# CrystalSixone/VLN-MAGIC

Measured on AMD Instinct MI355X. Metric: trajectory-steps/sec (whole node), MAGIC-S R2R pretrain, higher is better.
Workload: dtype bf16

## Files before the change

include/magic_hip.h:

```cpp
#ifndef MAGIC_HIP_H
#define MAGIC_HIP_H
#ifdef __cplusplus
extern "C" {
#endif

#define MAGIC_OK 0
#define MAGIC_ERR_ARG (-1)
#define MAGIC_ERR_LAUNCH (-2)
#define MAGIC_ERR_UNSUPPORTED (-3)

int magic_abi_version(void);
int magic_build_id(char* out, int len);
int magic_device_info(int* cu_count, int* clock_khz, char* arch, int arch_len);

int magic_gemm(int dtype, int layout, int batch, int nh, int M, int N, int K,
               const void* A, int lda, long long sAb, long long sAh,
               const void* B, int ldb, long long sBb, long long sBh,
               void* C, int ldc, long long sCb, long long sCh, int c_f32, int accumulate,
               const float* bias, int epilogue, const void* aux, int ldaux,
               const void* residual, int ldr, void* C2, int ldc2,
               float alpha, int splitk, float* bias_grad, void* stream);
int magic_gemm_set_big(int mode);
#define MAGIC_GEMM_FORM_PLAIN 0x1
#define MAGIC_GEMM_FORM_XCD 0x2
// ... 129 lines not shown
                      const float* dist, float* dsprel_w, float* dsprel_b, void* stream);
int magic_head_mean_fwd(int dtype, int B, int nh, long long inner, const void* P, float* out, void* stream);
int magic_head_mean_bwd(int B, int nh, long long inner, const float* g, float* dP, int accumulate, void* stream);

int magic_attn_supported(int dtype, int Nq, int Nk, int backward);
int magic_attn_fwd(int dtype, int B, int nh, int Nq, int Nk, const void* q, int ldq, const void* k, const void* v, int ldkv,
                   void* P, int ldp, void* ctx, int H, float scale, const unsigned char* kmask, const float* dist,
                   const float* sprel_w, const float* sprel_b,
                   const void* drop_seed, float drop_p, unsigned drop_site, void* Pd, void* stream);
int magic_attn_bwd(int dtype, int B, int nh, int Nq, int Nk, const void* q, int ldq, const void* k, const void* v, int ldkv,
                   const void* P, int ldp, const void* dctx, int H, float scale, const float* dP_init,
                   void* dq, int lddq, void* dk, void* dv, int lddkv,
                   const float* dist, float* dsprel_w, float* dsprel_b,
                   const void* drop_seed, float drop_p, unsigned drop_site, void* stream);
int magic_attn_bwd_ks(int dtype, int B, int nh, int Nq, int Nk, const void* q, int ldq, const void* k, const void* v, int ldkv,
                      const void* P, int ldp, const void* o, const void* dctx, int H, float scale,
                      void* dq, int lddq, void* dk, void* dv, int lddkv, int accumulate_kv,
                      const void* drop_seed, float drop_p, unsigned drop_site, void* stream);

int magic_lndot_fwd(int dtype, int M, int H, const void* Y, const float* gamma, const float* beta, float eps,
                    const float* w2, const float* b2, float* logit, void* stream);
int magic_lndot_bwd_blocks(int M);
int magic_lndot_bwd(int dtype, int M, int H, const void* Y, const float* gamma, const float* beta, float eps,
                    const float* w2, const float* dlogit, void* dZ, float* dgamma, float* dbeta, float* dw2, float* db2,
                    float* part, void* stream);

int magic_ce_rows(int dtype, int M, int N, const void* logits, int ld, const int* labels, int ignore_index,
                  float coef, const float* row_w, float* loss_row, void* dlogits, int ldd, int accumulate,
                  float* w_out, float w_rate, void* stream);
int magic_softkl_rows(int dtype, int M, int N, const void* logits, int ld, const float* targets, int ldt, float coef,
                      const float* row_w , float* loss_row, void* dlogits, int ldd,
                      void* stream);

int magic_kd_rows(int M, int N, const float* s, const float* t, int ld, float temperature, const float* w, float norm,
                  float coef, const float* coef_dev, float* loss_row, float* ds, int accumulate, void* stream);
int magic_kd_cols_parts(long long outer, int C, long long inner);
int magic_kd_cols(int dtype, long long outer, int C, long long inner, const void* s, long long s_stride, const void* t,
                  long long t_stride, float temperature, const float* w, float norm, float coef, float* loss_part, int n_parts,
                  void* ds, void* stream);
int magic_nav_act(int B, int K, const float* logits, int ld, const unsigned char* cand, int ldc, const unsigned char* mode,
                  const void* draws, float expl_max_ratio, int* action, float* stop_prob, float* entropy, void* stream);
int magic_mse(int dtype, int g_f32, long long outer, long long inner, const void* s, long long s_stride, const void* t,
              long long t_stride, const float* w, long long rows_per_w, float norm, float coef, const float* coef_dev, float* loss, void* ds,
              long long g_stride, int accumulate, void* stream);
typedef struct {
  int g_f32; long long outer, inner; const void* s; long long s_stride; const void* t; long long t_stride;
  const float* w; long long rows_per_w; float norm, coef; const float* coef_dev; float* loss; void* ds; long long g_stride; int accumulate;
  const int* valid_dev; const float* norm_dev; long long valid_mod;
} magic_mse_desc;
int magic_mse_multi(int dtype, int n, const magic_mse_desc* d, void* stream);
int magic_kd_emb_supported(int dtype, int Hs, int Ht);
int magic_kd_emb(int dtype, int n, const magic_mse_desc* d, int Hs, int Ht, const int* M, const void* const* W, const float* const* b,
                 void* const* d_acc, void* stream);
int magic_cfp_loss(int dtype, int B, int H, const void* a0, const void* a1, const void* a2, const void* txt, float temperature, float coef,
                   float* rows, void* d0, void* d1, void* d2, void* dtxt, float* part, int* counter, void* stream);

int magic_mlm_eval_supported(int dtype, int H);
int magic_mlm_eval_ws_need(int dtype, int nm, int V, int H);
int magic_mlm_eval(int dtype, int nm, int V, int H, const void* hm, const void* W, int ldw, const float* bias,
                   const int* labels, int ignore_index, void* ws, float* loss_row, int* hit_row, void* stream);
int magic_eval_rows(int dtype, int M, int N, const void* logits, int ld, const int* labels, int ignore_index,
                    const float* targets, int ldt, float* loss_row, int* hit_row, void* stream);
int magic_cfp_eval(int dtype, int B, int H, const void* a, const void* txt, float temperature,
                   float* loss_row, int* hit_row, void* stream);
int magic_eval_accum(int M, const float* loss_row, const int* hit_row, void* acc, int slot, void* stream);

int magic_csr_gather(int dtype, int n_out, int H, const void* src, const int* ptr, const int* idx, const float* w,
                     void* out, int accumulate, void* stream);
int magic_pano_fuse_fwd(int dtype, int N, int V, int H, const void* x, const int* lens, const float* wf, const float* bf,
                        void* fused, float* probs, const void* P, int nh, int inner, float* pmean, void* stream);
typedef struct {
  int B, K, Vp, use_gate;
  const float *g_raw, *l_raw, *fuse_raw; const unsigned char *gmask, *lmask; const int* fsrc; const unsigned char* bwmask;
  float *gl, *ll, *fl;
  const int *glab, *llab; int ignore_index; float coef;
  float *rows, *dgl, *dll, *dfl;
  const float* t_fused; float w_rate; int pad_; float* w_out;
  float T, kd_norm, kd_coef, pad2_; const float* kd_coef_dev; float* kd_rows;
} magic_sap_loss_params;
int magic_sap_fuse_loss(const void* params, int nbytes, void* stream);
int magic_pano_fuse_bwd_blocks(int N);
int magic_pano_fuse_bwd(int dtype, int N, int V, int H, const void* x, const float* probs, const float* wf, const void* dfused,
                        void* dx, float* dwf, float* dbf, void* stream);
int magic_sap_fuse_fwd(int B, int K, int Vp, const float* g_raw, const float* l_raw, const float* fuse_raw,
                       const unsigned char* gmask, const unsigned char* lmask, const int* fsrc, const unsigned char* bwmask,
                       int use_gate, float* gl, float* ll, float* fl, void* stream);
int magic_sap_fuse_bwd(int B, int K, int Vp, const float* g_raw, const float* l_raw, const float* fuse_raw,
                       const unsigned char* gmask, const unsigned char* lmask, const int* fsrc, const unsigned char* bwmask,
                       int use_gate, const float* dgl, const float* dll, const float* dfl,
                       float* dg_raw, float* dl_raw, float* dfuse_raw, void* stream);

int magic_step_rng(unsigned long long base_seed, unsigned* counter, float rw_temp, int* seed_out, float* rw_out, float* zero_me,
                   float* scale_state, float growth, float backoff, int interval, void* stream);
int magic_seed_scale(const float* scale_dev);
int magic_loss_assemble(const float* rows, int n_rows, const float* row_w, float row_scale, const float* kd_rows, int n_kd,
                        float* slots, const float* rw, float alpha, int has_kd, float* out, void* stream);

int magic_rowgate_fwd(int dtype, int M, int H, int mode, const void* x, const void* e, const float* wx, const float* we,
                      const float* b0, const float* b1, float* out_s, void* out, float* gsave, void* stream);
int magic_rowgate_bwd(int dtype, int M, int H, int mode, const void* x, const void* e, const float* wx, const float* we, const float* gsave,
                      const float* dy, const void* dout, void* dx, void* de, float* dwx, float* dwe, float* db0, float* db1, void* stream);

int magic_sumsq(long long n, const float* g, float* out, void* stream);
int magic_adamw(long long n, float* p, float* g, float* m, float* v, void* shadow, int shadow_dtype,
                float lr, float b1, float b2, float eps, float wd, float step_size,
                const float* sumsq, float max_norm, float gscale, const float* lr_ss, long long n_decay, int zero_grad,
                unsigned* overflow, float* scale_state, int* sched_step, int decay_first, void* stream);
int magic_sumsq_sched(long long n, const float* g, float* out, int* step, float lr0, int warmup, int total, float b1, float b2,
// ... 104 lines not shown
```

vln-magic_amd/csrc/loss.hip:

```cpp
#include "common.hpp"
#include <cstdint>

static const float* g_seed_scale = nullptr;
const float* seed_scale_get() { return g_seed_scale; }
extern "C" int magic_seed_scale(const float* scale_dev) { g_seed_scale = scale_dev; return MAGIC_OK; }

template <typename T>
__global__ __launch_bounds__(256) void ce_rows_kernel(int M, int N, const T* logits, int ld, const int* labels, int ignore_index,
                                                      float coef, const float* row_w, float* loss_row, T* dlogits, int ldd,
                                                      int accumulate, float* w_out, float w_rate, const float* ss) {
  __shared__ float red[8];
  if (ss) coef *= ss[0];
  const int row = blockIdx.x, tid = threadIdx.x, lane = tid & 63, wid = tid >> 6;
  const T* x = logits + (long long)row * ld;
  const int lab = labels[row];
  const bool ignored = (lab == ignore_index) || lab < 0 || lab >= N;
  const float xl = ignored ? 0.f : to_f(x[lab]);
  float mx = -3.0e38f;
  for (int c = tid; c < N; c += 256) mx = fmaxf(mx, to_f(x[c]));
  mx = wave_max(mx);
  if (lane == 0) red[wid] = mx;
  __syncthreads();
  mx = fmaxf(fmaxf(red[0], red[1]), fmaxf(red[2], red[3]));
  __syncthreads();
// ... 592 lines not shown
    const float sx = wave_sum(lane < B ? __expf(x - mx) : 0.f), sy = wave_sum(lane < B ? __expf(y - my) : 0.f);
    if (lane == 0) {
      const float lr = mx + __logf(sx), lc = my + __logf(sy);
      lse_r[r] = lr; lse_c[r] = lc;
      rows[(2 * pair) * B + r] = lr - sg[r][r];
      rows[(2 * pair + 1) * B + r] = lc - sg[r][r];
    }
  }
  if (!dtxt) return;
  __syncthreads();
#pragma unroll
  for (int j = 0; j < 4; ++j) {
    const int e = tid + 1024 * j, r = e >> 6, c = e & 63;
    float g = 0.f;
    if (r < B && c < B) {
      const float x = sg[r][c], d = r == c ? 1.f : 0.f;
      g = coef * ((__expf(x - lse_r[r]) - d) + (__expf(x - lse_c[c]) - d));
    }
    sg[r][c] = g;
  }
  __syncthreads();
  typedef __attribute__((ext_vector_type(2))) T vec2_t;
  const int hp = H >> 1;
  for (int o = tid; o < B * hp; o += 1024) {
    const int r = o / hp, h = (o - r * hp) * 2;
    float ga0 = 0.f, ga1 = 0.f, gt0 = 0.f, gt1 = 0.f;
#pragma unroll 8
    for (int q = 0; q < CFP_B; ++q) {
      const float g1 = sg[r][q], g2 = sg[q][r];
      const vec2_t t2 = *(const vec2_t*)(st + q * HS + h), a2v = *(const vec2_t*)(sa + q * HS + h);
      ga0 += g1 * to_f(t2[0]); ga1 += g1 * to_f(t2[1]);
      gt0 += g2 * to_f(a2v[0]); gt1 += g2 * to_f(a2v[1]);
    }
    da[(long long)r * H + h] = from_f<T>(ga0 * inv_temp); da[(long long)r * H + h + 1] = from_f<T>(ga1 * inv_temp);
    float* pp = part + (long long)pair * B * H + (long long)r * H + h;
    pp[0] = gt0; pp[1] = gt1;
  }
  __threadfence();
  __syncthreads();
  if (tid == 0) is_last = (atomicAdd(counter, 1) == 2) ? 1 : 0;
  __syncthreads();
  if (is_last) {
    __threadfence();
    for (int o = tid; o < B * H; o += 1024) {
      const float v = (__builtin_nontemporal_load(part + o) + __builtin_nontemporal_load(part + (long long)B * H + o)) + __builtin_nontemporal_load(part + 2ll * B * H + o);
      dtxt[o] = from_f<T>(v * inv_temp);
    }
    if (tid == 0) *counter = 0;
  }
}

static size_t cfp_lds_bytes(int H, int elt) { return (size_t)2 * CFP_B * (H + 16 / elt) * elt + 16 + (size_t)(CFP_B + 1) * (CFP_B + 1) * 4 + 2 * CFP_B * 4; }

extern "C" int magic_cfp_loss(int dtype, int B, int H, const void* a0, const void* a1, const void* a2, const void* txt, float temperature, float coef,
                              float* rows, void* d0, void* d1, void* d2, void* dtxt, float* part, int* counter, void* stream) {
  if (B <= 0 || B > CFP_B || H <= 0 || H > 256 || (H & 7) || !a0 || !a1 || !a2 || !txt || !rows || temperature <= 0.f) return MAGIC_ERR_ARG;
  if (((uintptr_t)a0 | (uintptr_t)a1 | (uintptr_t)a2 | (uintptr_t)txt) & 15) return MAGIC_ERR_ARG;
  if ((d0 == nullptr) != (d1 == nullptr) || (d0 == nullptr) != (d2 == nullptr) || (d0 == nullptr) != (dtxt == nullptr)) return MAGIC_ERR_ARG;
  if (dtxt && (!part || !counter)) return MAGIC_ERR_ARG;
  if (!dtype_ok(dtype)) return MAGIC_ERR_ARG;
  hipStream_t st = (hipStream_t)stream;
  const size_t shm = cfp_lds_bytes(H, dtype_is16(dtype) ? 2 : 4);
  static bool attr_set = false;
  if (!attr_set) {
    (void)hipFuncSetAttribute((const void*)cfp_loss_kernel<bf16>, hipFuncAttributeMaxDynamicSharedMemorySize, (int)cfp_lds_bytes(256, 2));
    (void)hipFuncSetAttribute((const void*)cfp_loss_kernel<f16>, hipFuncAttributeMaxDynamicSharedMemorySize, (int)cfp_lds_bytes(256, 2));
    (void)hipFuncSetAttribute((const void*)cfp_loss_kernel<float>, hipFuncAttributeMaxDynamicSharedMemorySize, (int)cfp_lds_bytes(256, 4));
    attr_set = true;
  }
  DISPATCH_T(dtype, hipLaunchKernelGGL(cfp_loss_kernel<TY>, dim3(3), dim3(1024), shm, st, B, H, (const TY*)a0, (const TY*)a1, (const TY*)a2, (const TY*)txt,
                                       1.f / temperature, coef, rows, (TY*)d0, (TY*)d1, (TY*)d2, (TY*)dtxt, part, counter, g_seed_scale));
  return launch_status();
}

extern "C" int magic_ce_rows(int dtype, int M, int N, const void* logits, int ld, const int* labels, int ignore_index,
                             float coef, const float* row_w, float* loss_row, void* dlogits, int ldd, int accumulate,
                             float* w_out, float w_rate, void* stream) {
  if (M <= 0 || N <= 0 || ld < N || (dlogits && ldd < N)) return MAGIC_ERR_ARG;
  dim3 grid(M), block(256);
  hipStream_t st = (hipStream_t)stream;
  const bool wide = dtype_is16(dtype) && N >= 2048 && !accumulate && (ld % 8) == 0 && (!dlogits || (ldd % 8) == 0) &&
                    (((uintptr_t)logits | (uintptr_t)dlogits) & 15) == 0;
  const bool big = M <= 512;
  if (wide)
    DISPATCH_H(dtype, DISPATCH_I2(big ? 1024 : 256, 1024, 256,
               hipLaunchKernelGGL((ce_rows_wide_kernel<TY, IV>), grid, dim3(IV), 0, st, M, N, (const TY*)logits, ld, labels, ignore_index, coef, row_w, loss_row, (TY*)dlogits, ldd, w_out, w_rate, g_seed_scale)));
  else
    DISPATCH_T(dtype, hipLaunchKernelGGL(ce_rows_kernel<TY>, grid, block, 0, st, M, N, (const TY*)logits, ld, labels, ignore_index, coef, row_w, loss_row, (TY*)dlogits, ldd, accumulate, w_out, w_rate, g_seed_scale));
  return launch_status();
}

extern "C" int magic_softkl_rows(int dtype, int M, int N, const void* logits, int ld, const float* targets, int ldt, float coef,
                                 const float* row_w, float* loss_row, void* dlogits, int ldd, void* stream) {
  if (M <= 0 || N <= 0 || ld < N || ldt < N || !logits || !targets || (dlogits && ldd < N) || dlogits == logits) return MAGIC_ERR_ARG;
  dim3 grid(M), block(256);
  hipStream_t st = (hipStream_t)stream;
  if (!dtype_ok(dtype)) return MAGIC_ERR_ARG;
  DISPATCH_T(dtype, hipLaunchKernelGGL(softkl_rows_kernel<TY>, grid, block, 0, st, M, N, (const TY*)logits, ld, targets, ldt, coef, row_w, loss_row, (TY*)dlogits, ldd, g_seed_scale));
  return launch_status();
}

extern "C" int magic_kd_rows(int M, int N, const float* s, const float* t, int ld, float temperature, const float* w, float norm,
                             float coef, const float* coef_dev, float* loss_row, float* ds, int accumulate, void* stream) {
  if (M <= 0 || N <= 0 || N > 512 || ld < N || temperature <= 0.f) return MAGIC_ERR_ARG;
  dim3 grid((M + 3) / 4), block(256);
  hipLaunchKernelGGL(kd_rows_kernel, grid, block, 0, (hipStream_t)stream, M, N, s, t, ld, temperature, w, norm, coef, coef_dev, loss_row, ds, accumulate, g_seed_scale);
  return launch_status();
}

static int kdc_cs(int C) { return C >= KDC_SPLIT_C ? 4 : 1; }

extern "C" int magic_kd_cols_parts(long long outer, int C, long long inner) {
  if (outer <= 0 || C <= 0 || inner <= 0) return MAGIC_ERR_ARG;
  long long n;
  if (inner < KDC_ROW_INNER) {
    n = (outer * inner + 3) / 4;
  } else {
    const long long gpb = 4 / kdc_cs(C);
    n = ((outer * inner + 63) / 64 + gpb - 1) / gpb;
  }
  return (int)(n < KDC_MAXB ? n : KDC_MAXB);
}

extern "C" int magic_kd_cols(int dtype, long long outer, int C, long long inner, const void* s, long long s_stride, const void* t,
// ... 220 lines not shown
```

vln-magic_amd/host/heads.py:

```python
import contextlib

import torch

from . import lib as _lib
from . import makd_pretrain as KD
from . import model_pretrain as MP
from . import ops as O
from .config import cfg_get
from .engine import rup


def cls_fwd(n, prefix, X, M, lda=None):
    l1 = n.lin(prefix + "net.0.weight")
    Y = O.linear_fwd(X, l1.W, l1.b, M, epilogue=2, lda=lda)
    return Y, cls_tail(n, prefix, Y, M)


def cls_tail(n, prefix, Y, M):
    ln, l2 = n.ln(prefix + "net.2"), n.lin(prefix + "net.3.weight")
    logit = n.new(M, dtype=torch.float32)
    O.lndot_fwd(Y, M, n.H, ln.g, ln.b, n.eps, l2.Wm, l2.b, logit)
    return logit


# ... 352 lines not shown
            O.lndot_bwd(Y, M, H, ln.g, ln.b, n.eps, l2.Wm, dlogit, dZh, ln.dg, ln.db, l2.dW, l2.db)
            O.linear_dw(dZh, X, l1.dW, l1.db, M)
            heads.append((dZh, l1, M, d_acc))
        with _lib.group():
            for dZh, l1, M, d_acc in heads:
                O.linear_dx(dZh, l1.W, M, out=d_acc, residual=d_acc)
        if c.use_gate:
            gate_fuse_bwd(n, "", c, df, B, K, Vp, c.d_gmap, c.d_vp, grouped=True)
        self._encoders_bwd(m, c)

    def metrics(self, m, c, block, temperature):
        plan = c.plan
        B, K, Vp = plan["B"], plan["K"], plan["Vp"]
        ga, la = plan["global_act_labels"], plan["local_act_labels"]
        for slot, (x, N, lab) in enumerate(((c.gl, K, ga), (c.ll, Vp, la), (c.fl, K, ga))):
            O.eval_accum(*O.eval_rows(x, B, N, N, labels=lab), B, block, slot)

    def result(self, m, c, o, batch):
        return dict(global_logits=c.gl, local_logits=c.ll, fused_logits=c.fl,
                    global_act_labels=m._dev(batch["global_act_labels"]), local_act_labels=m._dev(batch["local_act_labels"]))


class Cfp(_Glocal):
    def head(self, m, c, o, compute_loss, metrics):
        n, plan, B, L, K, Vp, H = _sizes(m, c)
        c.g0, c.v0, c.t0, c.gv0 = n.new(B, H), n.new(B, H), n.new(B, H), n.new(B, H)
        O.csr_gather_multi(H, [dict(out=c.g0, n_out=B, src1=c.glob.out, csr1=plan["g0"]),
                               dict(out=c.v0, n_out=B, src1=c.loc.out, csr1=plan["v0"]),
                               dict(out=c.t0, n_out=B, src1=c.txt_out, csr1=plan["t0"]),
                               dict(out=c.gv0, n_out=B, src1=c.glob.out, csr1=plan["g0"], src2=c.loc.out, csr2=plan["v0"])])
        with _lib.group():
            c.cfp = []
            for key, src in (("gmap", c.g0), ("vp", c.v0), ("fused", c.gv0), ("txt", c.t0)):
                hl = n.lin(f"cfp_heads.{key}.weight")
                c.cfp.append(O.linear_fwd(src, hl.W, hl.b, B))
        o["cfp"] = tuple(c.cfp)

    def rows(self, plan):
        B = plan["B"]
        return [B * plan["K"], B * plan["Vp"], B * plan["L"], B, B, B]

    def loss(self, m, c, o, zz, scg, kd):
        n, plan, B, L, K, Vp, H = _sizes(m, c)
        train = m.store.requires_grad
        c.d_gmap, c.d_vp, c.d_txt2 = zz(B * K, H), zz(B * Vp, H), zz(B * L, H)
        c.d_cls0 = (zz(B, H), zz(B, H), zz(B, H))
        temp = float(cfg_get(m.config, "cfp_temperature"))
        c.rows = n.new(6, B, dtype=torch.float32)
        txt_o = c.cfp[3]
        c.dsim, c.d_cfp = [], None
        ar = plan["arange_b"]
        lds = c.lds = rup(B, 8)
        fused = O.cfp_loss_ok(B, H)
        if fused:
            c.d_cfp = [n.new(B, H) for _ in range(4)] if train else None
            O.cfp_loss(B, H, c.cfp[:3], txt_o, temp, scg * 0.5 / B, c.rows, d_a=c.d_cfp[:3] if train else None, d_txt=c.d_cfp[3] if train else None)
        for i in (() if fused else range(3)):
            a = c.cfp[i]
            sim, simT = n.new(B, lds, dtype=torch.float32), n.new(B, lds, dtype=torch.float32)
            O.gemm(0, a, txt_o, sim, B, B, H, H, H, lds, alpha=1.0 / temp)
            O.gemm(0, txt_o, a, simT, B, B, H, H, H, lds, alpha=1.0 / temp)
            d1 = n.new(B, lds, dtype=torch.float32) if train else None
            d2 = n.new(B, lds, dtype=torch.float32) if train else None
            O.ce_rows(sim, B, B, lds, ar, coef=scg * 0.5 / B, loss_row=c.rows[2 * i], dlogits=d1, ldd=lds)
            O.ce_rows(simT, B, B, lds, ar, coef=scg * 0.5 / B, loss_row=c.rows[2 * i + 1], dlogits=d2, ldd=lds)
            c.dsim.append((d1, d2))
        c.temp = temp
        return c.rows, None, 0.5 / B

    def backward(self, m, c):
        n, plan, B, L, K, Vp, H = _sizes(m, c)
        d_outs = c.d_cfp if c.d_cfp is not None else [n.new(B, H) for _ in range(4)]
        txt_o = c.cfp[3]
        cast = lambda d: d if d.dtype == m.compute_dtype else O.cast_to(d, m.compute_dtype)
        for i in (() if c.d_cfp is not None else range(3)):
            d1, d2 = c.dsim[i]
            a = c.cfp[i]
            it = 1.0 / c.temp
            lds = c.lds
            e1, e2 = cast(d1), cast(d2)
            O.gemm(1, e1, txt_o, d_outs[i], B, H, B, lds, H, H, alpha=it)
            O.gemm(2, e2, txt_o, d_outs[i], B, H, B, lds, H, H, alpha=it, residual=d_outs[i], ldr=H)
            if i == 0:
                O.gemm(2, e1, a, d_outs[3], B, H, B, lds, H, H, alpha=it)
            else:
                O.gemm(2, e1, a, d_outs[3], B, H, B, lds, H, H, alpha=it, residual=d_outs[3], ldr=H)
            O.gemm(1, e2, a, d_outs[3], B, H, B, lds, H, H, alpha=it, residual=d_outs[3], ldr=H)
        d_g0, d_v0, d_t0 = c.d_cls0
        heads = list(zip((("gmap", c.g0, (d_g0,)), ("vp", c.v0, (d_v0,)), ("fused", c.gv0, (d_g0, d_v0)), ("txt", c.t0, (d_t0,))), d_outs))
        for (key, src, dsts), d_o in heads:
            hl = n.lin(f"cfp_heads.{key}.weight")
            O.linear_dw(d_o, src, hl.dW, hl.db, B)
        for sel in (("gmap", "vp", "txt"), ("fused",)):
            with _lib.group():
                for (key, src, dsts), d_o in heads:
                    if key in sel:
                        hl = n.lin(f"cfp_heads.{key}.weight")
                        for dst in dsts:
                            O.linear_dx(d_o, hl.W, B, out=dst, residual=dst)
        O.csr_gather_multi(H, [dict(out=c.d_gmap, n_out=B * K, accumulate=True, src1=d_g0, csr1=plan["g0_T"]),
                               dict(out=c.d_vp, n_out=B * Vp, accumulate=True, src1=d_v0, csr1=plan["v0_T"]),
                               dict(out=c.d_txt, n_out=B * L, accumulate=True, src1=d_t0, csr1=plan["t0_T"])])
        self._encoders_bwd(m, c)

    def metrics(self, m, c, block, temperature):
        temp = float(temperature if temperature is not None else cfg_get(m.config, "cfp_temperature"))
        for slot in range(3):
            O.eval_accum(*O.cfp_eval(c.cfp[slot], c.cfp[3], temp), c.plan["B"], block, slot)

    def result(self, m, c, o, batch):
        return o["cfp"]


UNITS = dict(mlm=Mlm(), mrc=Mrc(), sap=Sap(), cfp=Cfp())


def unit(task):
    if task not in UNITS:
        raise ValueError(task)
    return UNITS[task]
```

vln-magic_amd/host/ops.py:

```python
import contextlib
import ctypes as C
import os

import torch

from . import lanes
from . import lib as L

FLOPS = {"total": 0.0, "gemm": 0.0, "linear_ln": 0.0, "attn": 0.0, "enc": 0.0, "enabled": False}
BYTES = {"dw": 0.0, "dw_launches": 0}


def _flops(f, fam):
    if FLOPS["enabled"]:
        FLOPS["total"] += f
        FLOPS[fam] = FLOPS.get(fam, 0.0) + f


def _count(m, n, k, batch=1, fam="gemm"):
    _flops(2.0 * m * n * k * batch, fam)


_SUPPORTED = {}

# ... 955 lines not shown
                               L.P(q.get("valid_dev")), L.P(q.get("norm_dev")), int(q.get("valid_mod", 0)))
        L.call("magic_mse_multi", L.dt(dt0), len(chunk), arr, L.stream())
        i += len(chunk)


KD_FUSED = not os.environ.get("MAGIC_NO_KD_FUSED")


def kd_emb_ok(dtype, Hs, Ht):
    return KD_FUSED and dtype in L.HALF and bool(_supported("magic_kd_emb_supported", L.dt(dtype), int(Hs), int(Ht)))


def kd_emb(problems):
    i = 0
    while i < len(problems):
        chunk = problems[i:i + 8]
        n = len(chunk)
        W0 = chunk[0]["W"]
        Ht, Hs = W0.shape
        arr = (L.MseDesc * n)()
        Ms, Ws, bs, das = (C.c_int * n)(), (C.c_void_p * n)(), (C.c_void_p * n)(), (C.c_void_p * n)()
        for j, q in enumerate(chunk):
            s_, t_, W, ds, da, M = q["s"], q["t"], q["W"], q.get("ds"), q.get("d_acc"), int(q["M"])
            _chk(s_.dtype == t_.dtype == W.dtype == W0.dtype and tuple(W.shape) == (Ht, Hs) and W.stride(0) == Hs and W.stride(1) == 1, "kd_emb weights")
            _chk(q["b"].dtype == torch.float32 and q["b"].numel() >= Ht, "kd_emb bias")
            _chk(s_.is_contiguous() and t_.is_contiguous() and s_.numel() >= M * Hs and t_.numel() >= M * Ht, "kd_emb rows")
            _chk((ds is None) == (da is None), "kd_emb: ds and d_acc go together")
            _chk(ds is None or (ds.dtype == da.dtype == W.dtype and ds.is_contiguous() and da.is_contiguous() and ds.numel() >= M * Ht and da.numel() >= M * Hs),
                 "kd_emb gradients")
            inner = int(q["inner"])
            _chk(inner % Ht == 0 and int(q["outer"]) * (inner // Ht) == M, "kd_emb extents")
            arr[j] = L.MseDesc(0, q["outer"], inner, L.P(s_), (inner // Ht) * Hs, L.P(t_), inner, L.P(q.get("w")), q.get("rows_per_w", 1),
                               float(q.get("norm", 1.0)), float(q.get("coef", 0.0)), L.P(q.get("coef_dev")), L.P(q.get("loss")), L.P(ds), inner, 0,
                               L.P(q.get("valid_dev")), L.P(q.get("norm_dev")), 0)
            Ms[j], Ws[j], bs[j], das[j] = M, L.P(W), L.P(q["b"]), L.P(da)
            _count(M, Ht, Hs)
            if ds is not None:
                _count(M, Hs, Ht)
        L.call("magic_kd_emb", L.dt(W0.dtype), n, C.addressof(arr), Hs, Ht, C.addressof(Ms), C.addressof(Ws), C.addressof(bs), C.addressof(das), L.stream())
        i += n


def csr_gather(src, ptr, idx, w, out, n_out, H, accumulate=False):
    _chk(ptr.dtype == torch.int32 and idx.dtype == torch.int32 and ptr.numel() == n_out + 1, "csr arrays")
    L.call("magic_csr_gather", L.dt(src.dtype), n_out, H, L.P(src), L.P(ptr), L.P(idx), L.P(w), L.P(out), 1 if accumulate else 0,
           L.stream())


def cfp_loss_ok(B, H):
    return B <= 64 and H <= 256 and H % 8 == 0 and not os.environ.get("MAGIC_NO_FUSED_CFP")


_CFP_COUNTER = {}


def cfp_loss(B, H, a, txt, temperature, coef, rows, d_a=None, d_txt=None):
    _chk(len(a) == 3 and all(x.is_contiguous() and x.dtype == txt.dtype for x in a) and txt.is_contiguous(), "cfp_loss operands")
    d = d_a if d_a is not None else (None, None, None)
    part = cnt = None
    if d_txt is not None:
        part = torch.empty(3, B, H, dtype=torch.float32, device=txt.device)
        cnt = _CFP_COUNTER.get(txt.device)
        if cnt is None:
            cnt = _CFP_COUNTER[txt.device] = torch.zeros(1, dtype=torch.int32, device=txt.device)
    L.call("magic_cfp_loss", L.dt(txt.dtype), B, H, L.P(a[0]), L.P(a[1]), L.P(a[2]), L.P(txt), float(temperature), float(coef), L.P(rows),
           L.P(d[0]), L.P(d[1]), L.P(d[2]), L.P(d_txt), L.P(part), L.P(cnt), L.stream())


EVAL_FUSED = not os.environ.get("MAGIC_NO_EVAL_FUSED")
EVAL_BLOCK_BYTES = 96


def eval_block(device):
    return torch.zeros(EVAL_BLOCK_BYTES // 8, dtype=torch.int64, device=device)


def mlm_eval_ok(dtype, H):
    return EVAL_FUSED and dtype in L.HALF and bool(_supported("magic_mlm_eval_supported", L.dt(dtype), int(H)))


def _eval_out(M, device, loss_row, hit_row):
    loss_row = loss_row if loss_row is not None else torch.empty(M, dtype=torch.float32, device=device)
    hit_row = hit_row if hit_row is not None else torch.empty(M, dtype=torch.int32, device=device)
    _chk(loss_row.dtype == torch.float32 and hit_row.dtype == torch.int32 and loss_row.numel() >= M and hit_row.numel() >= M, "eval rows fp32 / int32 [M]")
    return loss_row, hit_row


def mlm_eval(hm, W, bias, labels, V, *, ignore_index=-1, loss_row=None, hit_row=None):
    nm, H = hm.shape
    _chk(hm.is_contiguous() and W.dtype == hm.dtype and W.stride(1) == 1 and W.shape[0] >= V and W.shape[1] == H, "mlm_eval operands")
    _chk(bias.dtype == torch.float32 and bias.numel() >= V and labels.dtype == torch.int32 and labels.numel() >= nm, "mlm_eval bias fp32 / labels int32")
    need = int(L.load().magic_mlm_eval_ws_need(L.dt(hm.dtype), nm, V, H))
    _chk(need > 0, "mlm_eval form")
    ws = torch.empty(need, dtype=torch.uint8, device=hm.device)
    loss_row, hit_row = _eval_out(nm, hm.device, loss_row, hit_row)
    L.call("magic_mlm_eval", L.dt(hm.dtype), nm, V, H, L.P(hm), L.P(W), W.stride(0), L.P(bias), L.P(labels), ignore_index, L.P(ws),
           L.P(loss_row), L.P(hit_row), L.stream())
    _count(nm, V, H)
    return loss_row, hit_row


def eval_rows(logits, M, N, ld, *, labels=None, ignore_index=-100, targets=None, loss_row=None, hit_row=None):
    _chk((labels is None) != (targets is None), "eval_rows: labels or targets")
    _chk(labels is None or (labels.dtype == torch.int32 and labels.numel() >= M), "eval_rows labels int32")
    _chk(targets is None or (targets.dtype == torch.float32 and targets.stride(-1) == 1), "eval_rows targets fp32")
    loss_row, hit_row = _eval_out(M, logits.device, loss_row, hit_row)
    L.call("magic_eval_rows", L.dt(logits.dtype), M, N, L.P(logits), ld, L.P(labels), ignore_index, L.P(targets),
           targets.stride(0) if targets is not None else 0, L.P(loss_row), L.P(hit_row), L.stream())
    return loss_row, hit_row


def cfp_eval(a, txt, temperature, *, loss_row=None, hit_row=None):
    B, H = txt.shape
    _chk(a.is_contiguous() and txt.is_contiguous() and a.dtype == txt.dtype and tuple(a.shape) == (B, H), "cfp_eval operands")
    loss_row, hit_row = _eval_out(B, txt.device, loss_row, hit_row)
    L.call("magic_cfp_eval", L.dt(txt.dtype), B, H, L.P(a), L.P(txt), float(temperature), L.P(loss_row), L.P(hit_row), L.stream())
    return loss_row, hit_row


# ... 220 lines not shown
```

Before: 202,700.

## Add MFMA bf16 CFP loss kernel with optional fused head input-gradient GEMMs

Adds a dedicated 16-bit CFP contrastive-loss kernel. It computes the similarity matrix and the gradient products with MFMA tiles and now handles every bf16/f16 call in place of the generic kernel. Behind the MAGIC_CFP_DX environment flag, the same kernel can also stage the four CFP head weights through a small ring of LDS slots and compute the heads' input gradients. The last block accumulates the shared fused and txt contributions, which removes the separate linear_dx launches. The fused path is off by default and adds LDS pressure, more serialized work in a three-block kernel, and a more complex cross-block completion protocol.

```diff
diff --git a/include/magic_hip.h b/include/magic_hip.h
--- a/include/magic_hip.h
+++ b/include/magic_hip.h
@@ -205,8 +205,9 @@
 int magic_kd_emb_supported(int dtype, int Hs, int Ht);
 int magic_kd_emb(int dtype, int n, const magic_mse_desc* d, int Hs, int Ht, const int* M, const void* const* W, const float* const* b,
                  void* const* d_acc, void* stream);
+int magic_cfp_loss_dx_supported(int dtype, int B, int H);
 int magic_cfp_loss(int dtype, int B, int H, const void* a0, const void* a1, const void* a2, const void* txt, float temperature, float coef,
-                   float* rows, void* d0, void* d1, void* d2, void* dtxt, float* part, int* counter, void* stream);
+                   float* rows, void* d0, void* d1, void* d2, void* dtxt, float* part, int* counter, const void* const* dx, int ldw, void* stream);
 
 int magic_mlm_eval_supported(int dtype, int H);
 int magic_mlm_eval_ws_need(int dtype, int nm, int V, int H);
diff --git a/profiles/micro/cfp_dx_probe.py b/profiles/micro/cfp_dx_probe.py
--- /dev/null
+++ b/profiles/micro/cfp_dx_probe.py
@@ -0,0 +1,78 @@
+import os
+import statistics
+import sys
+
+import torch
+
+sys.path.insert(0, os.path.join(os.path.dirname(os.path.abspath(__file__)), "..", ".."))
+import magic_amd
+from magic_amd.host import lib as L
+from magic_amd.host import ops as O
+
+B, H, ROUNDS, REPS = 48, 128, 9, 20
+DT = torch.bfloat16
+new = lambda: torch.empty(B, H, device="cuda", dtype=DT)
+a = [(0.5 * torch.randn(B, H, device="cuda")).to(DT) for _ in range(3)]
+txt = (0.5 * torch.randn(B, H, device="cuda")).to(DT)
+W = [(torch.randn(H, H, device="cuda") / H ** 0.5).to(DT) for _ in range(4)]
+rows = torch.empty(6, B, device="cuda")
+d_a, d_txt = [new() for _ in range(3)], new()
+d_cls = [torch.zeros(B, H, device="cuda", dtype=DT) for _ in range(3)]
+HAS_FUSED = hasattr(O, "cfp_loss_dx_ok")
+
+
+def loss():
+    O.cfp_loss(B, H, a, txt, 0.7, 0.37 / B, rows, d_a=d_a, d_txt=d_txt)
+
+
+def rows_only():
+    O.cfp_loss(B, H, a, txt, 0.7, 0.37 / B, rows)
+
+
+def sequence():
+    loss()
+    with L.group():
+        for d, w, dst in ((d_a[0], W[0], d_cls[0]), (d_a[1], W[1], d_cls[1]), (d_txt, W[3], d_cls[2])):
+            O.linear_dx(d, w, B, out=dst, residual=dst)
+    with L.group():
+        for dst in d_cls[:2]:
+            O.linear_dx(d_a[2], W[2], B, out=dst, residual=dst)
+
+
+def fused():
+    O.cfp_loss(B, H, a, txt, 0.7, 0.37 / B, rows, d_a=d_a, d_txt=d_txt, head_w=W, d_cls=d_cls)
+
+
+def graph_of(fn):
+    for _ in range(3):
+        fn()
+    g = torch.cuda.CUDAGraph()
+    with torch.cuda.graph(g):
+        for _ in range(REPS):
+            fn()
+    g.replay()
+    torch.cuda.synchronize()
+    return g
+
+
+def timed(g):
+    e0, e1 = torch.cuda.Event(enable_timing=True), torch.cuda.Event(enable_timing=True)
+    e0.record()
+    g.replay()
+    e1.record()
+    e1.synchronize()
+    return e0.elapsed_time(e1) * 1e3 / REPS
+
+
+forms = [("sequence", sequence), ("loss", loss), ("rows", rows_only)] + ([("fused", fused)] if HAS_FUSED else [])
+graphs = [(name, graph_of(fn)) for name, fn in forms]
+t = {name: [] for name, _ in forms}
+for _ in range(ROUNDS):
+    for name, g in graphs:
+        t[name].append(timed(g))
+print(f"B {B}, H {H}, bf16; {ROUNDS} rounds x {REPS} graph-replayed calls per form, interleaved; us per call")
+print("round  " + "  ".join(f"{name:>8s}" for name, _ in forms))
+for r in range(ROUNDS):
+    print(f"{r:5d}  " + "  ".join(f"{t[name][r]:8.2f}" for name, _ in forms))
+for name, _ in forms:
+    print(f"{name:9s} median {statistics.median(t[name]):6.2f}  min {min(t[name]):6.2f}")
diff --git a/vln-magic_amd/csrc/loss.hip b/vln-magic_amd/csrc/loss.hip
--- a/vln-magic_amd/csrc/loss.hip
+++ b/vln-magic_amd/csrc/loss.hip
@@ -668,24 +668,261 @@
 
 static size_t cfp_lds_bytes(int H, int elt) { return (size_t)2 * CFP_B * (H + 16 / elt) * elt + 16 + (size_t)(CFP_B + 1) * (CFP_B + 1) * 4 + 2 * CFP_B * 4; }
 
+#define CFP_WSLOTS 3
+#define CFP_SG_BYTES (((CFP_B + 1) * (CFP_B + 1) + 2 * CFP_B) * 4 + 12)
+static_assert(CFP_SG_BYTES % 16 == 0, "the weight slots behind sg stay 16-byte aligned");
+__host__ __device__ static inline int cfp_hp(int H) { return (H + 31) & ~31; }
+__host__ __device__ static inline int cfp_kc(int H) { return cfp_hp(H) <= 128 ? cfp_hp(H) : 32; }
+struct CfpDx { const void* W[4]; void* d_g0; void* d_v0; void* d_t0; int ldw; };
+static size_t cfp16_lds_bytes(int H, bool dx) {
+  return (size_t)2 * CFP_B * (cfp_hp(H) + 8) * 2 + CFP_SG_BYTES + (dx ? (size_t)CFP_WSLOTS * cfp_kc(H) * (H + 8) * 2 : 0);
+}
+
+template <typename Hh>
+__global__ __launch_bounds__(1024) void cfp_loss16_kernel(int B, int H, const Hh* a0, const Hh* a1, const Hh* a2, const Hh* txt, float inv_temp, float coef,
+                                                          float* rows, Hh* d0, Hh* d1, Hh* d2, Hh* dtxt, float* part, int* counter, const float* ss,
+                                                          CfpDx dx, int has_dx) {
+  extern __shared__ __attribute__((aligned(16))) unsigned char cfp_smem[];
+  if (ss) coef *= ss[0];
+  typedef rowvec<Hh> vec_t;
+  typedef __attribute__((ext_vector_type(4))) unsigned u32x4;
+  const int Hp = cfp_hp(H), HS = Hp + 8, Bp = (B + 15) & ~15, nb = Bp >> 4;
+  const int KC = cfp_kc(H), nkc = Hp / KC, WP = H + 8;
+  Hh* sa = (Hh*)cfp_smem;
+  Hh* st = sa + CFP_B * HS;
+  float (*sg)[CFP_B + 1] = (float (*)[CFP_B + 1])(st + CFP_B * HS);
+  float* lse_r = &sg[CFP_B][0];
+  float* lse_c = lse_r + CFP_B;
+  Hh* sw = (Hh*)((unsigned char*)(st + CFP_B * HS) + CFP_SG_BYTES);
+  __shared__ int is_last;
+  const int tid = threadIdx.x, lane = tid & 63, wave = tid >> 6, pair = blockIdx.x;
+  const int lr = lane & 15, lg = lane >> 4;
+  const Hh* a = pair == 0 ? a0 : pair == 1 ? a1 : a2;
+  Hh* da = pair == 0 ? d0 : pair == 1 ? d1 : d2;
+  const int nstage = has_dx ? nkc * (pair < 2 ? 3 : 2) : 0;
+  auto wimg = [&](int s) {
+    const int wi = s / nkc, kc = s - wi * nkc, widx = pair < 2 ? (wi == 0 ? pair : wi + 1) : wi + 2;
+    RowImg<Hh> im;
+    im.s = sw + (s % CFP_WSLOTS) * KC * WP; im.pitch = WP;
+    const void* W = widx == 0 ? dx.W[0] : widx == 1 ? dx.W[1] : widx == 2 ? dx.W[2] : dx.W[3];
+    im.src = (const Hh*)W + (long long)kc * KC * dx.ldw; im.ld = dx.ldw;
+    im.nvalid = H - kc * KC; im.cvalid = H; im.cpr = H >> 3; im.nchunk = KC * im.cpr;
+    return im;
+  };
+  int w_loaded = nstage < CFP_WSLOTS ? nstage : CFP_WSLOTS;
+  vec_t rw[CFP_WSLOTS][2];
+  {
+    RowImg<Hh> ia, it;
+    ia.s = sa; ia.pitch = HS; ia.src = a; ia.ld = H; ia.nvalid = B; ia.cvalid = H; ia.cpr = Hp >> 3; ia.nchunk = Bp * ia.cpr;
+    it = ia; it.s = st; it.src = txt;
+    vec_t ra[2], rt[2];
+    stage_issue<2>(ra, ia, 0, tid, 1024);
+    stage_issue<2>(rt, it, 0, tid, 1024);
+#pragma unroll
+    for (int u = 0; u < CFP_WSLOTS; ++u) if (u < w_loaded) stage_issue<2>(rw[u], wimg(u), 0, tid, 1024);
+    stage_store<2>(ra, ia, 0, tid, 1024);
+    stage_store<2>(rt, it, 0, tid, 1024);
+  }
+  __syncthreads();
+  if (wave < nb * nb) {
+    const int tr = wave / nb, tc = wave - tr * nb;
+    f32x4 acc = {0.f, 0.f, 0.f, 0.f};
+    for (int k0 = 0; k0 < Hp; k0 += 32) acc = mfma16(frag_kc<Hh>(sa, HS, 16 * tr, k0, lane), frag_kc<Hh>(st, HS, 16 * tc, k0, lane), acc);
+#pragma unroll
+    for (int i = 0; i < 4; ++i) sg[16 * tr + 4 * lg + i][16 * tc + lr] = acc[i] * inv_temp;
+  }
+  __syncthreads();
+  for (int r = wave; r < B; r += 16) {
+    const float x = lane < B ? sg[r][lane] : -3.0e38f, y = lane < B ? sg[lane][r] : -3.0e38f;
+    const float mx = wave_max(x), my = wave_max(y);
+    const float sx = wave_sum(lane < B ? __expf(x - mx) : 0.f), sy = wave_sum(lane < B ? __expf(y - my) : 0.f);
+    if (lane == 0) {
+      const float lrw = mx + __logf(sx), lcw = my + __logf(sy);
+      lse_r[r] = lrw; lse_c[r] = lcw;
+      rows[(2 * pair) * B + r] = lrw - sg[r][r];
+      rows[(2 * pair + 1) * B + r] = lcw - sg[r][r];
+    }
+  }
+  if (!dtxt) return;
+  __syncthreads();
+#pragma unroll
+  for (int j = 0; j < 4; ++j) {
+    const int e = tid + 1024 * j, r = e >> 6, c = e & 63;
+    float g = 0.f;
+    if (r < B && c < B) {
+      const float x = sg[r][c], d = r == c ? 1.f : 0.f;
+      g = coef * ((__expf(x - lse_r[r]) - d) + (__expf(x - lse_c[c]) - d));
+    }
+    sg[r][c] = g;
+  }
+  __syncthreads();
+  const int nct = Hp >> 4, ntile = nb * nct;
+  f32x4 acc_a[4];
+#pragma unroll
+  for (int j = 0; j < 4; ++j) {
+    const int t = wave + 16 * j;
+    acc_a[j] = f32x4{0.f, 0.f, 0.f, 0.f};
+    if (t < ntile) {
+      const int rt = t / nct, ct = t - rt * nct;
+      f32x4 acc_t = {0.f, 0.f, 0.f, 0.f};
+#pragma unroll 4
+      for (int k0 = 0; k0 < Bp; k0 += 4) {
+        const int k = k0 + lg, col = 16 * ct + lr;
+        acc_a[j] = mfma16(sg[16 * rt + lr][k], to_f(st[k * HS + col]), acc_a[j]);
+        acc_t = mfma16(sg[k][16 * rt + lr], to_f(sa[k * HS + col]), acc_t);
+      }
+#pragma unroll
+      for (int i = 0; i < 4; ++i) {
+        const int r = 16 * rt + 4 * lg + i, c = 16 * ct + lr;
+        if (r < B && c < H) part[(long long)pair * B * H + (long long)r * H + c] = acc_t[i];
+      }
+    }
+  }
+  __syncthreads();
+#pragma unroll
+  for (int j = 0; j < 4; ++j) {
+    const int t = wave + 16 * j;
+    if (t < ntile) {
+      const int rt = t / nct, ct = t - rt * nct;
+#pragma unroll
+      for (int i = 0; i < 4; ++i) {
+        const int r = 16 * rt + 4 * lg + i, c = 16 * ct + lr;
+        const Hh v = from_f<Hh>(acc_a[j][i] * inv_temp);
+        sa[r * HS + c] = v;
+        if (r < B && c < H) da[(long long)r * H + c] = v;
+      }
+    }
+  }
+#pragma unroll
+  for (int u = 0; u < CFP_WSLOTS; ++u) if (u < w_loaded) stage_store<2>(rw[u], wimg(u), 0, tid, 1024);
+  const int nctw = H >> 4, ntw = nb * nctw;
+  auto w_acquire = [&](int s) {
+    if (s >= w_loaded) {
+      __syncthreads();
+      vec_t rq[CFP_WSLOTS][2];
+#pragma unroll
+      for (int u = 0; u < CFP_WSLOTS; ++u) if (s + u < nstage) stage_issue<2>(rq[u], wimg(s + u), 0, tid, 1024);
+#pragma unroll
+      for (int u = 0; u < CFP_WSLOTS; ++u) if (s + u < nstage) stage_store<2>(rq[u], wimg(s + u), 0, tid, 1024);
+      w_loaded = s + CFP_WSLOTS < nstage ? s + CFP_WSLOTS : nstage;
+      __syncthreads();
+    }
+    return (const Hh*)(sw + (s % CFP_WSLOTS) * KC * WP);
+  };
+  auto dx_mm = [&](f32x4 (&acc)[4], const Hh* sx, int s0) {
+#pragma unroll
+    for (int j = 0; j < 4; ++j) acc[j] = f32x4{0.f, 0.f, 0.f, 0.f};
+    for (int kc = 0; kc < nkc; ++kc) {
+      const Hh* w = w_acquire(s0 + kc);
+#pragma unroll
+      for (int j = 0; j < 4; ++j) {
+        const int t = wave + 16 * j;
+        if (t < ntw) {
+          const int rt = t / nctw, ct = t - rt * nctw;
+          for (int k0 = 0; k0 < KC; k0 += 32)
+            acc[j] = mfma16(frag_kc<Hh>(sx, HS, 16 * rt, kc * KC + k0, lane), frag_oc<Hh>(w, WP, 16 * ct, k0, lane), acc[j]);
+        }
+      }
+    }
+  };
+  auto dx_out = [&](const f32x4 (&acc)[4], auto&& put) {
+#pragma unroll
+    for (int j = 0; j < 4; ++j) {
+      const int t = wave + 16 * j;
+      if (t < ntw) {
+        const int rt = t / nctw, ct = t - rt * nctw;
+#pragma unroll
+        for (int i = 0; i < 4; ++i) {
+          const int r = 16 * rt + 4 * lg + i;
+          if (r < B) put(r * H + 16 * ct + lr, acc[j][i]);
+        }
+      }
+    }
+  };
+  auto ld16 = [](const Hh* p) { return __builtin_bit_cast(Hh, __builtin_nontemporal_load((const unsigned short*)p)); };
+  f32x4 acc_x[4];
+  if (has_dx && pair < 2) {
+    __syncthreads();
+    dx_mm(acc_x, sa, 0);
+    Hh* dst = (Hh*)(pair == 0 ? dx.d_g0 : dx.d_v0);
+    dx_out(acc_x, [&](int o, float v) { dst[o] = from_f<Hh>(v); });
+  }
+  asm volatile("s_waitcnt vmcnt(0)" ::: "memory");
+  __syncthreads();
+  if (tid == 0) {
+    __builtin_amdgcn_fence(__ATOMIC_RELEASE, "agent");
+    asm volatile("s_waitcnt vmcnt(0)" ::: "memory");
+    is_last = (atomicAdd(counter, 1) == 2) ? 1 : 0;
+    if (is_last) {
+      __builtin_amdgcn_fence(__ATOMIC_ACQUIRE, "agent");
+      asm volatile("s_waitcnt vmcnt(0)" ::: "memory");
+    }
+  }
+  __syncthreads();
+  if (is_last) {
+    for (int o = tid; o < B * H; o += 1024) {
+      const float v = (__builtin_nontemporal_load(part + o) + __builtin_nontemporal_load(part + (long long)B * H + o)) + __builtin_nontemporal_load(part + 2ll * B * H + o);
+      const Hh hv = from_f<Hh>(v * inv_temp);
+      dtxt[o] = hv;
+      if (has_dx) { const int r = o / H; st[r * HS + (o - r * H)] = hv; }
+    }
+    if (has_dx) {
+      if (pair != 2) {
+        const int cpr = H >> 3;
+        for (int i = tid; i < B * cpr; i += 1024) {
+          const int r = i / cpr, c = (i - r * cpr) * 8;
+          *(u32x4*)(sa + r * HS + c) = __builtin_nontemporal_load((const u32x4*)(d2 + (long long)r * H + c));
+        }
+      }
+      __syncthreads();
+      Hh* dg = (Hh*)dx.d_g0; Hh* dv = (Hh*)dx.d_v0; Hh* dt = (Hh*)dx.d_t0;
+      dx_mm(acc_x, sa, pair < 2 ? nkc : 0);
+      dx_out(acc_x, [&](int o, float v) { dg[o] = from_f<Hh>(to_f(ld16(dg + o)) + v); dv[o] = from_f<Hh>(to_f(ld16(dv + o)) + v); });
+      dx_mm(acc_x, st, pair < 2 ? 2 * nkc : nkc);
+      dx_out(acc_x, [&](int o, float v) { dt[o] = from_f<Hh>(v); });
+    }
+    if (tid == 0) *counter = 0;
+  }
+}
+
+extern "C" int magic_cfp_loss_dx_supported(int dtype, int B, int H) {
+  return dtype_is16(dtype) && B >= 1 && B <= CFP_B && H >= 16 && H <= 256 && (H & 15) == 0;
+}
+
 extern "C" int magic_cfp_loss(int dtype, int B, int H, const void* a0, const void* a1, const void* a2, const void* txt, float temperature, float coef,
-                              float* rows, void* d0, void* d1, void* d2, void* dtxt, float* part, int* counter, void* stream) {
+                              float* rows, void* d0, void* d1, void* d2, void* dtxt, float* part, int* counter, const void* const* dx, int ldw, void* stream) {
   if (B <= 0 || B > CFP_B || H <= 0 || H > 256 || (H & 7) || !a0 || !a1 || !a2 || !txt || !rows || temperature <= 0.f) return MAGIC_ERR_ARG;
   if (((uintptr_t)a0 | (uintptr_t)a1 | (uintptr_t)a2 | (uintptr_t)txt) & 15) return MAGIC_ERR_ARG;
   if ((d0 == nullptr) != (d1 == nullptr) || (d0 == nullptr) != (d2 == nullptr) || (d0 == nullptr) != (dtxt == nullptr)) return MAGIC_ERR_ARG;
   if (dtxt && (!part || !counter)) return MAGIC_ERR_ARG;
   if (!dtype_ok(dtype)) return MAGIC_ERR_ARG;
+  CfpDx dxv = {};
+  if (dx) {
+    if (!magic_cfp_loss_dx_supported(dtype, B, H)) return MAGIC_ERR_UNSUPPORTED;
+    if (!dtxt || ldw < H || (ldw & 7)) return MAGIC_ERR_ARG;
+    uintptr_t al = (uintptr_t)d2;
+    for (int i = 0; i < 7; ++i) if (!dx[i]) return MAGIC_ERR_ARG;
+    for (int i = 0; i < 4; ++i) { dxv.W[i] = dx[i]; al |= (uintptr_t)dx[i]; }
+    if (al & 15) return MAGIC_ERR_ARG;
+    dxv.d_g0 = (void*)dx[4]; dxv.d_v0 = (void*)dx[5]; dxv.d_t0 = (void*)dx[6]; dxv.ldw = ldw;
+  }
   hipStream_t st = (hipStream_t)stream;
-  const size_t shm = cfp_lds_bytes(H, dtype_is16(dtype) ? 2 : 4);
   static bool attr_set = false;
   if (!attr_set) {
-    (void)hipFuncSetAttribute((const void*)cfp_loss_kernel<bf16>, hipFuncAttributeMaxDynamicSharedMemorySize, (int)cfp_lds_bytes(256, 2));
-    (void)hipFuncSetAttribute((const void*)cfp_loss_kernel<f16>, hipFuncAttributeMaxDynamicSharedMemorySize, (int)cfp_lds_bytes(256, 2));
+    size_t most = 0;
+    for (int h = 8; h <= 256; h += 8) most = most > cfp16_lds_bytes(h, true) ? most : cfp16_lds_bytes(h, true);
+    (void)hipFuncSetAttribute((const void*)cfp_loss16_kernel<bf16>, hipFuncAttributeMaxDynamicSharedMemorySize, (int)most);
+    (void)hipFuncSetAttribute((const void*)cfp_loss16_kernel<f16>, hipFuncAttributeMaxDynamicSharedMemorySize, (int)most);
     (void)hipFuncSetAttribute((const void*)cfp_loss_kernel<float>, hipFuncAttributeMaxDynamicSharedMemorySize, (int)cfp_lds_bytes(256, 4));
     attr_set = true;
   }
-  DISPATCH_T(dtype, hipLaunchKernelGGL(cfp_loss_kernel<TY>, dim3(3), dim3(1024), shm, st, B, H, (const TY*)a0, (const TY*)a1, (const TY*)a2, (const TY*)txt,
-                                       1.f / temperature, coef, rows, (TY*)d0, (TY*)d1, (TY*)d2, (TY*)dtxt, part, counter, g_seed_scale));
+  if (dtype_is16(dtype))
+    DISPATCH_H(dtype, hipLaunchKernelGGL(cfp_loss16_kernel<TY>, dim3(3), dim3(1024), cfp16_lds_bytes(H, dx != nullptr), st, B, H, (const TY*)a0, (const TY*)a1,
+                                         (const TY*)a2, (const TY*)txt, 1.f / temperature, coef, rows, (TY*)d0, (TY*)d1, (TY*)d2, (TY*)dtxt, part, counter,
+                                         g_seed_scale, dxv, dx ? 1 : 0));
+  else
+    hipLaunchKernelGGL(cfp_loss_kernel<float>, dim3(3), dim3(1024), cfp_lds_bytes(H, 4), st, B, H, (const float*)a0, (const float*)a1, (const float*)a2,
+                       (const float*)txt, 1.f / temperature, coef, rows, (float*)d0, (float*)d1, (float*)d2, (float*)dtxt, part, counter, g_seed_scale);
   return launch_status();
 }
 
diff --git a/vln-magic_amd/host/heads.py b/vln-magic_amd/host/heads.py
--- a/vln-magic_amd/host/heads.py
+++ b/vln-magic_amd/host/heads.py
@@ -428,9 +428,11 @@
         ar = plan["arange_b"]
         lds = c.lds = rup(B, 8)
         fused = O.cfp_loss_ok(B, H)
+        c.cfp_dx = fused and train and O.cfp_loss_dx_ok(txt_o.dtype, B, H)
         if fused:
             c.d_cfp = [n.new(B, H) for _ in range(4)] if train else None
-            O.cfp_loss(B, H, c.cfp[:3], txt_o, temp, scg * 0.5 / B, c.rows, d_a=c.d_cfp[:3] if train else None, d_txt=c.d_cfp[3] if train else None)
+            dx = dict(head_w=[n.lin(f"cfp_heads.{k}.weight").W for k in ("gmap", "vp", "fused", "txt")], d_cls=c.d_cls0) if c.cfp_dx else {}
+            O.cfp_loss(B, H, c.cfp[:3], txt_o, temp, scg * 0.5 / B, c.rows, d_a=c.d_cfp[:3] if train else None, d_txt=c.d_cfp[3] if train else None, **dx)
         for i in (() if fused else range(3)):
             a = c.cfp[i]
             sim, simT = n.new(B, lds, dtype=torch.float32), n.new(B, lds, dtype=torch.float32)
@@ -467,7 +469,7 @@
         for (key, src, dsts), d_o in heads:
             hl = n.lin(f"cfp_heads.{key}.weight")
             O.linear_dw(d_o, src, hl.dW, hl.db, B)
-        for sel in (("gmap", "vp", "txt"), ("fused",)):
+        for sel in (() if c.cfp_dx else (("gmap", "vp", "txt"), ("fused",))):
             with _lib.group():
                 for (key, src, dsts), d_o in heads:
                     if key in sel:
diff --git a/vln-magic_amd/host/ops.py b/vln-magic_amd/host/ops.py
--- a/vln-magic_amd/host/ops.py
+++ b/vln-magic_amd/host/ops.py
@@ -1031,9 +1031,14 @@
 
 
 _CFP_COUNTER = {}
-
-
-def cfp_loss(B, H, a, txt, temperature, coef, rows, d_a=None, d_txt=None):
+CFP_DX = bool(os.environ.get("MAGIC_CFP_DX"))
+
+
+def cfp_loss_dx_ok(dtype, B, H):
+    return CFP_DX and dtype in L.HALF and bool(_supported("magic_cfp_loss_dx_supported", L.dt(dtype), B, H))
+
+
+def cfp_loss(B, H, a, txt, temperature, coef, rows, d_a=None, d_txt=None, *, head_w=None, d_cls=None):
     _chk(len(a) == 3 and all(x.is_contiguous() and x.dtype == txt.dtype for x in a) and txt.is_contiguous(), "cfp_loss operands")
     d = d_a if d_a is not None else (None, None, None)
     part = cnt = None
@@ -1042,8 +1047,16 @@
         cnt = _CFP_COUNTER.get(txt.device)
         if cnt is None:
             cnt = _CFP_COUNTER[txt.device] = torch.zeros(1, dtype=torch.int32, device=txt.device)
+    dx = None
+    if head_w is not None or d_cls is not None:
+        _chk(head_w is not None and d_cls is not None and len(head_w) == 4 and len(d_cls) == 3 and d_txt is not None, "cfp_loss head gradients: four weights, three destinations, the gradient form")
+        _chk(all(w.dtype == txt.dtype and tuple(w.shape) == (H, H) and w.stride(1) == 1 and w.stride(0) == head_w[0].stride(0) for w in head_w), "cfp_loss head weights")
+        _chk(all(t.dtype == txt.dtype and t.is_contiguous() and t.numel() >= B * H for t in d_cls), "cfp_loss head gradient destinations")
+        dx = (C.c_void_p * 7)(*[t.data_ptr() for t in list(head_w) + list(d_cls)])
+        for _ in range(5):
+            _count(B, H, H)
     L.call("magic_cfp_loss", L.dt(txt.dtype), B, H, L.P(a[0]), L.P(a[1]), L.P(a[2]), L.P(txt), float(temperature), float(coef), L.P(rows),
-           L.P(d[0]), L.P(d[1]), L.P(d[2]), L.P(d_txt), L.P(part), L.P(cnt), L.stream())
+           L.P(d[0]), L.P(d[1]), L.P(d[2]), L.P(d_txt), L.P(part), L.P(cnt), C.addressof(dx) if dx is not None else None, head_w[0].stride(0) if dx is not None else 0, L.stream())
 
 
 EVAL_FUSED = not os.environ.get("MAGIC_NO_EVAL_FUSED")
```

Result: no change. 202,400 (median of 2 runs) (-0.2%).
